# wg-perception/tod

Measured on AMD Instinct MI355X. Metric: frames/sec @ 640x480, 1M-descriptor DB; achieved HBM GB/s on BF-matcher, higher is better.
Workload: dtype fp4 (+-1) x fp4 -> f32 on the matrix cores (exact integers), f32 in the verifier

## Files before the change

tod_amd/csrc/orb.hip:

```cpp
#include <algorithm>
#include <cstring>
#include <vector>

#include "ctx.h"
#include "orb_arc.h"
#include "orb_compass.h"
#include "orb_stages.h"

using namespace tod_orb;

namespace {

#include "orb_pyramid.h"
#include "orb_fast.h"
#include "orb_select.h"
#include "orb_describe.h"

struct OrbGraph {
  struct Key { uint32_t H, W, n_features, n_levels, cap, F; float sf; const void *kp, *aux, *desc, *img0, *mask, *taps; } key = {};
  hipGraph_t graph = nullptr;
  hipGraphExec_t exec = nullptr;
  void drop() {
    if (exec) (void)hipGraphExecDestroy(exec);
    if (graph) (void)hipGraphDestroy(graph);
// ... 37 lines not shown
  TOD_HIP(ws->o_desc.reserve((size_t)P.F * P.cap * 32));
  if (masked) TOD_HIP(ws->maskbuf.reserve(P.F * P.px));
  TOD_HIP(ws->taps.reserve((size_t)P.n_taps * sizeof(ResizeTap) + 32));
  return TODHIP_OK;
}

int upload_pattern(todhip_ctx* ctx, OrbWs* ws, const int8_t* pattern) {
  if (!pattern && ws->pattern_is_default) return TODHIP_OK;
  int8_t hpat[1024];
  if (pattern) std::memcpy(hpat, pattern, 1024); else default_pattern(hpat);
  ws->pattern_is_default = !pattern;
  TOD_HIP(hipMemcpyAsync(ws->pattern.p, hpat, 1024, hipMemcpyHostToDevice, ctx->stream));
  TOD_HIP(hipStreamSynchronize(ctx->stream));
  return TODHIP_OK;
}

int upload_taps(todhip_ctx* ctx, OrbWs* ws, const OrbPlan& P, float scale_factor) {
  const OrbWs::TapsFor now = {P.H, P.W, P.n_levels, scale_factor, ws->taps.p};
  if (std::memcmp(&now, &ws->taps_for, sizeof(now)) == 0 || P.n_taps == 0u) return TODHIP_OK;
  std::vector<ResizeTap> taps(P.n_taps);
  fill_resize_taps(P, taps.data());
  TOD_HIP(hipMemcpyAsync(ws->taps.p, taps.data(), taps.size() * sizeof(ResizeTap), hipMemcpyHostToDevice, ctx->stream));
  TOD_HIP(hipStreamSynchronize(ctx->stream));
  ws->taps_for = now;
  return TODHIP_OK;
}

void record_stages(const OrbPlan& P, const OrbWs* ws, const uint8_t* d_mask, hipStream_t st) {
  const LevelTab& T = P.tab;
  const size_t px = P.px;
  for (uint32_t lvl = 1; lvl < P.n_levels; ++lvl) {
    if (P.resize_x[lvl] == 0u) continue;
    uint8_t* img = ws->pyr.as<uint8_t>() + (size_t)lvl * P.F * px;
    const ResizeTap* taps = ws->taps.as<ResizeTap>();
    hipLaunchKernelGGL(resize_kernel, grid(P.resize[lvl]), dim3(256), 0, st, img - (size_t)P.F * px, T.w[lvl - 1], img, T.h[lvl], T.w[lvl],
                       taps + P.tap_x[lvl], taps + P.tap_y[lvl], px);
  }
  uint32_t* ctl = ws->small.as<uint32_t>();
  uint32_t* level_counts = ctl + P.level_counts_off;
  Cand* cand = ws->cand.as<Cand>(); Cand* eq = ws->eq.as<Cand>(); Cand* sel1 = ws->sel1.as<Cand>(); Cand* sel2 = ws->sel2.as<Cand>();
  hipLaunchKernelGGL(fast_nms_kernel, grid(P.fast_nms), dim3(256), 0, st, T, cand, P.cand_cap, ctl, ctl + W_HIST, d_mask, P.H, P.W, px);
  hipLaunchKernelGGL(fast_threshold_kernel, grid(P.fast_threshold), dim3(64), 0, st, T, ctl, P.cand_cap);
  hipLaunchKernelGGL(split_kernel, grid(P.split), dim3(256), 0, st, T, cand, ctl, sel1, eq, P.cand_cap, P.sel1_cap);
  hipLaunchKernelGGL(rank_tiled_kernel, grid(P.rank_ties), dim3(256), 0, st, RankArgs::rank_ties(eq, P.cand_cap, sel1, P.sel1_cap, ctl));
  hipLaunchKernelGGL(harris_kernel, grid(P.harris), dim3(256), 0, st, T, sel1, ctl + W_NSEL1, px, P.sel1_cap);
  hipLaunchKernelGGL(rank_tiled_kernel, grid(P.rank_harris), dim3(256), 0, st,
                     RankArgs::rank_harris(sel1, P.sel1_cap, sel2, P.sel2_cap, ctl, level_counts, P.F));
  hipLaunchKernelGGL(blur_kernel, grid(P.blur), dim3(256), 0, st, T, ws->blur.as<uint8_t>(), px);
  DescribeArgs D;
  std::memset(&D, 0, sizeof(D));
  disc_umax(D.umax);
  D.blur = ws->blur.as<uint8_t>(); D.sel = sel2; D.level_counts = level_counts; D.cap = P.cap; D.pattern = ws->pattern.as<int8_t>();
  D.kp_xy = ws->o_xy.as<float>(); D.kp_aux = ws->o_aux.as<float>(); D.desc = ws->o_desc.as<uint8_t>(); D.fs = px; D.sel_fs = P.sel2_cap;
  hipLaunchKernelGGL(describe_kernel, grid(P.describe), dim3(256), 0, st, T, D);
}

int orb_device(todhip_ctx* ctx, const OrbIn& in, const OrbParams& par, const OrbOut& out) {
  OrbPlan P;
  if (const int bad = orb_plan(in.F, in.H, in.W, par.n_features, par.n_levels, par.scale_factor, out.cap, &P)) return bad;
  OrbWs* ws = tod_ws<OrbWs>(ctx);
  hipStream_t st = ctx->stream;
  if (P.want_max == 0) {
    ws->graph.drop();
    ws->plan = P;
    for (uint32_t f = 0; f < in.F; ++f) out.n_out[f] = 0;
    TOD_HIP(hipStreamSynchronize(st));
    return TODHIP_OK;
  }
  if (const int rc = reserve_buffers(ctx, ws, P, in.d_mask != nullptr)) return rc;
  if (const int rc = upload_pattern(ctx, ws, par.pattern)) return rc;
  if (const int rc = upload_taps(ctx, ws, P, par.scale_factor)) return rc;
  for (uint32_t lvl = 0; lvl < P.n_levels; ++lvl) P.tab.img[lvl] = ws->pyr.as<uint8_t>() + (size_t)lvl * P.F * P.px;
  ws->plan = P;
  uint32_t* ctl = ws->small.as<uint32_t>();
  TOD_HIP(hipMemsetAsync(ctl, 0, P.ctl_words * sizeof(uint32_t), st));
  if (in.stride == P.W && (P.F == 1 || in.gray_fs == P.px))
    TOD_HIP(hipMemcpyAsync(ws->pyr.p, in.d_gray, (size_t)P.F * P.px, hipMemcpyDeviceToDevice, st));
  else
    hipLaunchKernelGGL(copy_rows_kernel, grid(P.copy_rows), dim3(256), 0, st, in.d_gray, in.stride, ws->pyr.as<uint8_t>(), P.H, P.W,
                       in.gray_fs, P.px);
  const uint8_t* ws_mask = nullptr;
  if (in.d_mask) {
    ws_mask = ws->maskbuf.as<uint8_t>();
    hipLaunchKernelGGL(copy_rows_kernel, grid(P.copy_rows), dim3(256), 0, st, in.d_mask, P.W, ws->maskbuf.as<uint8_t>(), P.H, P.W, P.px, P.px);
  }
  float* const ws_xy = ws->o_xy.as<float>(); float* const ws_aux = ws->o_aux.as<float>(); uint8_t* const ws_desc = ws->o_desc.as<uint8_t>();
  static const bool use_graph = getenv("TODHIP_ORB_NO_GRAPH") == nullptr;
  if (!use_graph) {
    record_stages(ws->plan, ws, ws_mask, st);
  } else {
    const OrbGraph::Key key = {P.H, P.W, par.n_features, P.n_levels, P.cap, P.F, par.scale_factor, ws_xy, ws_aux, ws_desc, ws->pyr.p, ws_mask, ws->taps.p};
    if (!ws->graph.matches(key)) {
      TOD_HIP(ws->graph.begin_capture(st));
      record_stages(ws->plan, ws, ws_mask, st);
      TOD_HIP(ws->graph.end_capture(st, key));
    }
    TOD_HIP(ws->graph.launch(st));
  }
  uint32_t* d_totals = ctl + P.totals_off;
  hipLaunchKernelGGL(copy_out_kernel, grid(P.copy_out), dim3(256), 0, st, ctl + P.level_counts_off, P.n_levels, P.cap, ws_xy, ws_aux,
                     reinterpret_cast<const uint32_t*>(ws_desc), out.kp_xy, out.kp_aux, reinterpret_cast<uint32_t*>(out.desc), d_totals);
  TOD_HIP(hipGetLastError());
  uint32_t* h_totals = ws->h_out.as<uint32_t>();
  TOD_HIP(hipMemcpyAsync(h_totals, d_totals, (size_t)P.F * sizeof(uint32_t), hipMemcpyDeviceToHost, st));
  TOD_HIP(hipStreamSynchronize(st));
  for (uint32_t f = 0; f < P.F; ++f) out.n_out[f] = std::min(h_totals[f], P.cap);
  return TODHIP_OK;
// ... 113 lines not shown
```

tod_amd/csrc/orb_describe.h:

```cpp

struct DescribeArgs {
  const uint8_t* blur;
  const Cand* sel;
  const uint32_t* level_counts;
  uint32_t cap;
  const int8_t* pattern; int umax[kHalfPatch + 2];
  float* kp_xy; float* kp_aux; uint8_t* desc;
  size_t fs; uint32_t sel_fs;
};

__global__ __launch_bounds__(256) void describe_kernel(LevelTab T, const DescribeArgs A) {
  const uint32_t v = blockIdx.y, lvl = v / T.F, f = v - lvl * T.F;
  if (T.want[lvl] == 0u) return;
  const uint8_t* __restrict__ img = T.img[lvl] + f * A.fs;
  const uint8_t* __restrict__ blur = A.blur + v * A.fs;
  const Cand* __restrict__ sel = A.sel + (size_t)v * A.sel_fs;
  const uint32_t* __restrict__ level_counts = A.level_counts + f * kCtlWords;
  float* kp_xy = A.kp_xy + (size_t)f * A.cap * 2; float* kp_aux = A.kp_aux + (size_t)f * A.cap * 4;
  uint8_t* desc = A.desc + (size_t)f * A.cap * 32;
  const float scale = T.scale[lvl];
  const uint32_t i = blockIdx.x * 4u + (threadIdx.x >> 6), l = threadIdx.x & 63u;
  if (i >= level_counts[lvl]) return;
  uint32_t base = 0;
  for (uint32_t j = 0; j < lvl; ++j) base += level_counts[j];
  const uint32_t o = base + i;
  if (o >= A.cap) return;
  const Cand c = sel[i];
  const int x = c.x, y = c.y, W = (int)T.w[lvl];
  int m10, m01;
  patch_moments(img, W, x, y, A.umax, l, m10, m01);
  const float fm10 = (float)m10, fm01 = (float)m01;
  float ca, sa;
  steer_of(fm10, fm01, ca, sa);
  uint32_t nib = 0;
#pragma unroll
  for (int b = 0; b < 4; ++b) nib |= (uint32_t)steered_test(blur, W, x, y, ca, sa, A.pattern + 4 * (4 * (int)l + b)) << b;
  const uint32_t hi = __shfl_down(nib, 1);
  if ((l & 1u) == 0u) desc[(size_t)o * 32 + (l >> 1)] = (uint8_t)(nib | (hi << 4));
  if (l == 0) {
    float ang = atan2f(fm01, fm10) * 57.29577951308232f;
    if (ang < 0.f) ang += 360.f;
    kp_xy[2 * o] = (float)x * scale; kp_xy[2 * o + 1] = (float)y * scale;
    kp_aux[4 * o] = 31.f * scale; kp_aux[4 * o + 1] = ang; kp_aux[4 * o + 2] = c.harris; kp_aux[4 * o + 3] = (float)lvl;
  }
}

__global__ __launch_bounds__(256) void copy_out_kernel(const uint32_t* __restrict__ level_counts, uint32_t n_levels, uint32_t cap,
                                                       const float* __restrict__ s_xy, const float* __restrict__ s_aux,
                                                       const uint32_t* __restrict__ s_desc, float* __restrict__ d_xy,
                                                       float* __restrict__ d_aux, uint32_t* __restrict__ d_desc,
                                                       uint32_t* __restrict__ totals) {
  const uint32_t f = blockIdx.y;
  level_counts += f * kCtlWords;
  s_xy += (size_t)f * cap * 2; s_aux += (size_t)f * cap * 4; s_desc += (size_t)f * cap * 8;
  d_xy += (size_t)f * cap * 2; d_aux += (size_t)f * cap * 4; d_desc += (size_t)f * cap * 8;
  uint32_t total = 0;
  for (uint32_t l = 0; l < n_levels; ++l) total += level_counts[l];
  const uint32_t n = min(total, cap);
  const uint32_t i = blockIdx.x * 256u + threadIdx.x;
  if (i == 0) totals[f] = total;
  if (i < 2u * n) d_xy[i] = s_xy[i];
  if (i < 4u * n) d_aux[i] = s_aux[i];
  if (i < 8u * n) d_desc[i] = s_desc[i];
}
```

tod_amd/csrc/orb_stages.h:

```cpp
#pragma once

#include "ctx.h"
#include "orb_moments.h"
#include "orb_plan.h"

namespace tod_orb {

__device__ __forceinline__ uint32_t wave_append(uint32_t* counter, bool flag) {
  const uint32_t lane = threadIdx.x & 63u;
  const unsigned long long bal = __builtin_amdgcn_ballot_w64(flag);
  if (bal == 0ull) return 0u;
  const uint32_t first = (uint32_t)__ffsll((long long)bal) - 1u;
  uint32_t base = 0;
  if (lane == first) base = atomicAdd(counter, (uint32_t)__popcll(bal));
  base = (uint32_t)__builtin_amdgcn_readlane((int)base, (int)first);
  return base + (uint32_t)__popcll(bal & ((1ull << lane) - 1ull));
}

__device__ __forceinline__ uint32_t wave_prefix_sum(uint32_t v) {
#define TOD_ORB_DPP_ADD(ctrl, rows) v += (uint32_t)__builtin_amdgcn_update_dpp(0, (int)v, ctrl, rows, 0xF, false)
  TOD_ORB_DPP_ADD(0x111, 0xF); TOD_ORB_DPP_ADD(0x112, 0xF); TOD_ORB_DPP_ADD(0x114, 0xF); TOD_ORB_DPP_ADD(0x118, 0xF);
  TOD_ORB_DPP_ADD(0x142, 0xA); TOD_ORB_DPP_ADD(0x143, 0xC);
#undef TOD_ORB_DPP_ADD
  return v;
}
__device__ __forceinline__ uint32_t wave_sum(uint32_t v) { return (uint32_t)__builtin_amdgcn_readlane((int)wave_prefix_sum(v), 63); }

__device__ __forceinline__ void patch_moments(const uint8_t* __restrict__ img, int W, int x, int y, const int (&umax)[kHalfPatch + 2],
                                              uint32_t l, int& m10, int& m01) {
  m10 = 0; m01 = 0;
  if (l < 31u) {
    const int v = (int)l - kHalfPatch;
    const int d = v == 0 ? kHalfPatch : umax[v < 0 ? -v : v];
    int rs;
    row_moments(img + (size_t)(y + v) * W + x - kHalfPatch, d, rs, m10);
    m01 = v * rs;
  }
  m10 = (int)wave_sum((uint32_t)m10); m01 = (int)wave_sum((uint32_t)m01);
}

__device__ __forceinline__ void steer_of(float fm10, float fm01, float& ca, float& sa) {
  const float nrm = sqrtf(fm10 * fm10 + fm01 * fm01);
  ca = nrm > 0.f ? fm10 / nrm : 1.f; sa = nrm > 0.f ? fm01 / nrm : 0.f;
}

__device__ __forceinline__ bool steered_test(const uint8_t* __restrict__ blur, int W, int x, int y, float ca, float sa, const int8_t* pp) {
  const int x0 = (int)rintf((float)pp[0] * ca - (float)pp[1] * sa), y0 = (int)rintf((float)pp[0] * sa + (float)pp[1] * ca);
  const int x1 = (int)rintf((float)pp[2] * ca - (float)pp[3] * sa), y1 = (int)rintf((float)pp[2] * sa + (float)pp[3] * ca);
  const int t0 = blur[(uint32_t)(y + y0) * (uint32_t)W + (uint32_t)(x + x0)], t1 = blur[(uint32_t)(y + y1) * (uint32_t)W + (uint32_t)(x + x1)];
  return t0 < t1;
}

struct Stages {
  LevelTab T;
  const uint8_t* blur; const Cand* sel; const uint32_t* level_counts;
  size_t fs; uint32_t sel_fs, want_max, n;
  int umax[kHalfPatch + 2];
};

}

int tod_orb_stage_host_view(todhip_ctx* ctx, const uint8_t* gray, const uint8_t* mask, uint32_t H, uint32_t W, uint32_t stride,
                            const uint8_t** d_gray, const uint8_t** d_mask);
int tod_orb_stages(todhip_ctx* ctx, const uint8_t* d_gray, const uint8_t* d_mask, uint32_t H, uint32_t W, uint32_t stride,
                   uint32_t n_features, uint32_t n_levels, float scale_factor, tod_orb::Stages* out);
```

tod_amd/csrc/verify.hip:

```cpp
#include <algorithm>
#include <chrono>
#include <atomic>
#include <climits>
#include <cmath>
#include <cstdio>
#include <cstdlib>
#include <cstring>
#include <limits>
#include <map>
#include <memory>
#include <mutex>
#include <thread>
#include <vector>

#include "ctx.h"
#include "depth_rescale.h"
#include "verify_kernels.h"
#include "verify_draw_bits.h"

using namespace tod;

namespace {

#include "verify_launch.h"
#include "verify_prep.h"
#include "verify_draw.h"
#include "verify_clique.h"
#include "verify_eval.h"
#include "verify_growth.h"
#include "verify_sprint.h"


struct VerifyWs {
  DevBuf train, query, qidx, kpxy, phys, samp, bits, sampdeg, nvalid, table, iter_samples, counts, gate_m,
      small, deferred, stacks, kp_bits, clique_adj, adjc_scratch, c_kept, c_offs, c_qpt, c_obj, c_hist, c_goff,
      sprint_status, sprint_stack, c_src, c_cnt;
  HostBuf m_small, m_hist, m_pos, m_counts, m_kp, m_nvalid;
  HostBuf m_sprint, m_sprint_out, m_sprint_kp;
  HostBuf h_small;
};

struct StreamCache;
struct VerifyPool : TodWs {
  static constexpr int kSlot = kWsVerify;
  std::vector<VerifyWs*> slots; std::vector<StreamCache*> streams;
  std::vector<hipEvent_t> side_ev;
  static constexpr size_t kMaxLanes = 17;
  HostBuf args_stage[kMaxLanes]; DevBuf args_dev[kMaxLanes];
  DevBuf kceil; bool kceil_ready = false;
  ~VerifyPool() override;
};
struct SideStreams {
  struct PerDevice {
    std::vector<hipStream_t> st;
    std::atomic<bool> taken[16];
    uint32_t partition = 0;
    PerDevice() { for (auto& t : taken) t.store(false); }
  };
  std::mutex mu;
  std::map<int, PerDevice> by_device;
  hipError_t get(int device, uint32_t n, std::vector<hipStream_t>& out, PerDevice** pd) {
    std::lock_guard<std::mutex> g(mu);
    PerDevice& d = by_device[device];
    const uint32_t part = tod_cu_partition();
    if (d.partition != part) {
      bool in_use = false;
      for (size_t i = 0; i < d.st.size(); ++i) in_use = in_use || d.taken[i].load();
      if (!in_use) {
        for (hipStream_t s0 : d.st) { (void)hipStreamSynchronize(s0); (void)hipStreamDestroy(s0); }
        d.st.clear();
        d.partition = part;
// ... 410 lines not shown
```

tod_amd/csrc/verify_engine.h:

```cpp

enum Phase { PH_CLUSTER, PH_CLUSTER_WAIT, PH_PREPALL, PH_PREPALL_WAIT, PH_OBJECT, PH_ROUND, PH_PREP_WAIT, PH_DRAW,
             PH_DRAW_WAIT, PH_EVAL2, PH_EVAL2_WAIT, PH_GROWTH, PH_GROWTH_WAIT, PH_SPRINT_WAIT, PH_DONE };

struct RoundState {
  uint64_t consumed = 0;
  uint32_t it_drawn = 0, attempts_carry = 0;
  bool selection_empty = false, loop_done = false;
  int iterations = 0, n_best = -INT_MAX;
  double k = 1.0;
  uint32_t best_it = 0;
  uint64_t pos_after_stop = 0;
  uint32_t batch = 16, lookahead = 4096;
  uint32_t nvalid = 0, total_iters = 0;
  uint32_t it_begin = 0, want = 0, got = 0, S = 0, window_len = 0;
  uint32_t n_def = 0;
  uint32_t s_floor = 0;
};

inline uint64_t sprint_margin0() {
  static const uint64_t v = [] { const char* e = getenv("TODHIP_SPRINT_MARGIN"); const long long x = e ? atoll(e) : 0; return x > 0 ? (uint64_t)x : (uint64_t)(1u << 17); }();
  return v;
}
struct Slot {
  VerifyWs* ws = nullptr;
// ... 574 lines not shown
        for (uint32_t i = 0; i < n; ++i) { const dim3 e = extent(host[start[c] + i0 + i]); gx = std::max(gx, e.x); gy = std::max(gy, e.y); }
        const dim3 grid = slot_dim == 1 ? dim3(gx, n) : dim3(gx, gy, n);
        SlotsPtr<A> S = {dev + start[c] + i0};
        hipLaunchKernelGGL(kern, grid, dim3(block), lds, st, S);
      }
    }
    return true;
  }

  struct Staging { bool ok = false; size_t used = 0; };
  template <uint32_t N, class A, class KernP, class KernV, class Extent>
  void launch_either(hipStream_t st, KernP kern_ptr, KernV kern_val, const std::vector<A>& v, bool long_list, Staging& stage, int slot_dim,
                     Extent extent, uint32_t block, uint32_t lds, bool by_class) {
    if (long_list && stage.ok && launch_many(st, kern_ptr, v, slot_dim, extent, stage.used, block, lds, by_class)) return;
    launch_list<N>(st, kern_val, v, block, lds, slot_dim, extent);
  }
#define TOD_BOTH_FORMS(kern, A, N) kern<SlotsPtr<A>>, kern<Slots<A, N>>

  template <class F>
  static void split_evals(const std::vector<EvalArgs>& v, uint32_t lds, bool deferred, F& launch_evals) {
    bool any_wide = false, any_narrow = false;
    for (const EvalArgs& a : v) (a.job.W <= 8u ? any_narrow : any_wide) = true;
    if (any_wide && any_narrow) { launch_evals(v, true, lds, deferred); return; }
    launch_evals(v, any_wide, lds, deferred);
  }
  void launch_all(hipStream_t st) {
    Staging stage;
    {
      const size_t n_eval = L.eval_small.size() + L.eval_direct.size() + L.eval_big.size();
      if (L.adj.size() > 4u * kManySlots || n_eval > kMaxSlots || L.prep_small.size() > kManySlots) {
        VerifyPool* pool = tod_ws<VerifyPool>(ctx);
        const size_t need = L.finite.size() * sizeof(JobArgs) + L.adj.size() * sizeof(AdjArgs) + L.prep.size() * sizeof(PrepArgs) +
                            L.prep_small.size() * sizeof(PrepSmallArgs) + n_eval * sizeof(EvalArgs) + 4096u;
        stage.ok = pool->args_stage[lane_now].reserve(need) == hipSuccess && pool->args_dev[lane_now].reserve(need) == hipSuccess;
      }
    }
    auto launch_evals = [&](const std::vector<EvalArgs>& v, bool wide, uint32_t lds, bool deferred) {
      pick_eval(wide, deferred, [&](auto kern_ptr, auto kern_val, auto ext) {
        launch_either<kMaxSlots>(st, kern_ptr, kern_val, v, v.size() > kMaxSlots, stage, 1, ext, 64u, lds, false);
      });
    };
    auto words = [](const CopyArgs& a) { return dim3(std::max(1u, std::min(64u, (a.n + 255u) / 256u))); };
    L.copy_in.insert(L.copy_in.end(), L.zero.begin(), L.zero.end());
    launch_list<kCopySlots>(st, copy_words_kernel, L.copy_in, 256, 0, 1, words);
    for (size_t i = 0; i < L.sprint.size(); ++i) { L.sprint[i].rnd = L.sprint_src[i]->dev.as<uint32_t>(); L.sprint[i].rnd_len = L.sprint_src[i]->dev_valid; }
    launch_list<kWideSlots>(st, sprint_kernel, L.sprint, kSprintThreads, kSprintLds, 0, [](const SprintArgs&) { return dim3(1); });
    launch_list(st, cluster_frame_kernel, L.cluster, 256, 0, 0, [](const ClusterArgs&) { return dim3(1); });
    launch_list(st, cluster_frame_rescaled_kernel, L.cluster_rescaled, 256, 0, 0, [](const ClusterRescaledArgs&) { return dim3(1); });
    launch_list<kWideSlots>(st, invalidate_kernel, L.inval, 256, 0, 0, [](const InvArgs&) { return dim3(1); });
    launch_either<kManySlots>(st, TOD_BOTH_FORMS(small_prep_kernel, PrepSmallArgs, kManySlots), L.prep_small, L.prep_small.size() > kManySlots, stage,
                              1, [](const PrepSmallArgs&) { return dim3(1); }, 64u, 0u, false);
    {
      auto ext_rows = [](const auto& a) { return dim3((a.job.n + 255u) / 256u); };
      auto ext_adj = [](const AdjArgs& a) { return dim3(a.job.n, (a.job.W + 3u) / 4u); };
      const bool many = L.adj.size() > 4u * kManySlots;
      launch_either<kManySlots>(st, TOD_BOTH_FORMS(finite_kernel, JobArgs, kManySlots), L.finite, many, stage, 1, ext_rows, 256u, 0u, true);
      launch_either<kManySlots>(st, TOD_BOTH_FORMS(adjacency_kernel, AdjArgs, kManySlots), L.adj, many, stage, 2, ext_adj, 256u, 0u, true);
      launch_either<kManySlots>(st, TOD_BOTH_FORMS(round_prep_kernel, PrepArgs, kManySlots), L.prep, many, stage, 1, ext_rows, 256u, 0u, true);
    }
    for (int f = DRAW_FORMS - 1; f >= 0; --f) {
      for (size_t i = 0; i < L.draw[f].size(); ++i) L.draw[f][i].rnd = L.draw_src[f][i].first->dev.as<uint32_t>() + L.draw_src[f][i].second;
      launch_draws(st, (DrawForm)f, L.draw[f]);
    }
    {
      uint32_t lds = 0;
      for (const ChainArgs& c : L.chain) lds = std::max(lds, (std::min(c.S, kChainLdsEntries) + std::min(c.n_req, kChainMaxReq)) * 4u);
      launch_list<kWideSlots>(st, chain_kernel, L.chain, 256, lds, 0, [](const ChainArgs&) { return dim3(1); });
    }
    {
      uint32_t lds = 8192u;
      for (const EvalArgs& a : L.eval_small) lds = std::max(lds, a.lds_bytes);
      for (EvalArgs& a : L.eval_small) a.lds_bytes = lds;
      split_evals(L.eval_small, lds, false, launch_evals);
    }
    split_evals(L.eval_direct, kEvalLdsBig, false, launch_evals);
    split_evals(L.eval_big, kEvalLdsBig, true, launch_evals);
    launch_list(st, growth_kernel, L.growth, 256, 0, 0, [](const GrowthArgs&) { return dim3(1); });
    launch_list<kWideSlots>(st, invalidate_kernel, L.inval_after, 256, 0, 0, [](const InvArgs&) { return dim3(1); });
    launch_list<kManySlots>(st, round_prep_kernel<Slots<PrepArgs, kManySlots>>, L.prep_after, 256, 0, 1, [](const PrepArgs& a) { return dim3((a.job.n + 255u) / 256u); });
    launch_list<kCopySlots>(st, copy_words_kernel, L.copy_out, 256, 0, 1, words);
    L = Launches();
  }
#undef TOD_BOTH_FORMS

  int run(std::vector<Slot*>& slots) {
    std::vector<StreamCache*>& caches = tod_ws<VerifyPool>(ctx)->streams;
    for (Slot* s : slots) {
      s->start_draws = s->rng->draws; s->abs_pos = 0; s->stream = nullptr;
      for (StreamCache* c : caches) if (c->same_start(*s->rng)) { s->stream = c; break; }
      if (!s->stream) {
        if (caches.size() >= 64) {
          bool in_use = false;
          for (Slot* t : slots) in_use = in_use || t->stream == caches.front();
          if (!in_use) { TOD_HIP(hipStreamSynchronize(st)); caches.front()->dev.release(); delete caches.front(); caches.erase(caches.begin()); }
        }
        caches.push_back(new StreamCache(*s->rng));
        s->stream = caches.back();
      }
    }
    const int rc_run = run_ticks(slots);
    for (Slot* s : slots) {
      if (s->abs_pos) { const uint64_t d0 = s->start_draws; *s->rng = s->stream->state_at(s->abs_pos); s->rng->draws = d0 + s->abs_pos; }
      s->stream = nullptr;
    }
    return rc_run;
  }
  static constexpr uint32_t kHeavyN = 96;
  enum Kind { K_LIGHT = 0, K_GROWTH = 1, K_SPRINT = 2, K_EVAL = 3, K_COUNT = 4 };
  static Kind kind_of(const Slot& s) {
    if (s.ph == PH_OBJECT) {
// ... 119 lines not shown
```

tod_amd/csrc/verify_hooks.h:

```cpp

namespace {
struct LookupArgs { const float* kp_xy; const void* depth; float* z; uint32_t* err; uint32_t n, H, W; int is_u16, rescale; RescaleGeom geom; };
__global__ __launch_bounds__(256) void depth_lookup_kernel(LookupArgs a) {
  const uint32_t q = blockIdx.x * 256u + threadIdx.x;
  if (q >= a.n) return;
  const int row = (int)a.kp_xy[2 * q + 1], col = (int)a.kp_xy[2 * q];
  if (row < 0 || col < 0 || (uint32_t)row >= a.H || (uint32_t)col >= a.W) { atomicExch(a.err, 1u); return; }
  a.z[q] = a.rescale ? rescaled_depth_at(a.depth, a.is_u16, a.geom, (uint32_t)col, (uint32_t)row)
                     : depth_metres(a.depth, a.is_u16, (size_t)row * a.W + col);
}
__global__ __launch_bounds__(64) void kabsch_test_kernel(uint32_t n, const double* Hd, const float* C, float* R, float* T) {
  const uint32_t i = blockIdx.x * 64u + threadIdx.x;
  if (i >= n) return;
  double h[9]; float c[6], r[9], t[3];
  for (int k = 0; k < 9; ++k) h[k] = Hd[(size_t)i * 9 + k];
  for (int k = 0; k < 6; ++k) c[k] = C[(size_t)i * 6 + k];
  kabsch_solve(h, c, r, t);
  for (int k = 0; k < 9; ++k) R[(size_t)i * 9 + k] = r[k];
  for (int k = 0; k < 3; ++k) T[(size_t)i * 3 + k] = t[k];
}
}

extern "C" {

int todhip_test_kabsch(todhip_ctx* ctx, uint32_t n_cases, const double* Hd, const float* C, float* R, float* T) {
  if (!ctx || !Hd || !C || !R || !T || n_cases == 0 || n_cases > (1u << 20)) return TODHIP_EINVAL;
  TOD_HIP(hipSetDevice(ctx->device));
  VerifyWs* ws = ws_of(ctx);
  hipStream_t st = ctx->stream;
  const size_t n = n_cases;
  TOD_HIP(ws->phys.reserve(n * 9 * sizeof(double))); TOD_HIP(ws->train.reserve(n * 6 * sizeof(float)));
  TOD_HIP(ws->query.reserve(n * 9 * sizeof(float))); TOD_HIP(ws->kpxy.reserve(n * 3 * sizeof(float)));
  TOD_HIP(hipMemcpyAsync(ws->phys.p, Hd, n * 9 * sizeof(double), hipMemcpyHostToDevice, st));
  TOD_HIP(hipMemcpyAsync(ws->train.p, C, n * 6 * sizeof(float), hipMemcpyHostToDevice, st));
  hipLaunchKernelGGL(kabsch_test_kernel, dim3((n_cases + 63u) / 64u), dim3(64), 0, st, n_cases, ws->phys.as<double>(),
                     ws->train.as<float>(), ws->query.as<float>(), ws->kpxy.as<float>());
  TOD_HIP(hipGetLastError());
  TOD_HIP(hipMemcpyAsync(R, ws->query.p, n * 9 * sizeof(float), hipMemcpyDeviceToHost, st));
  TOD_HIP(hipMemcpyAsync(T, ws->kpxy.p, n * 3 * sizeof(float), hipMemcpyDeviceToHost, st));
  TOD_HIP(hipStreamSynchronize(st));
  return TODHIP_OK;
}

int todhip_test_adjacency(todhip_ctx* ctx, const float* train, const float* query, const float* kpxy, uint32_t n,
                          float span, float err, uint64_t* phys, uint64_t* samp) {
  if (!ctx || !train || !query || !kpxy || !phys || !samp || n == 0 || n > (uint32_t)kMaxWords * 64u) return TODHIP_EINVAL;
  TOD_HIP(hipSetDevice(ctx->device));
  VerifyWs* ws = ws_of(ctx);
  const uint32_t W = (n + 63u) / 64u;
  hipStream_t st = ctx->stream;
  TOD_HIP(ws->train.reserve((size_t)n * 12)); TOD_HIP(ws->query.reserve((size_t)n * 12));
  TOD_HIP(ws->kpxy.reserve((size_t)n * 8));
  TOD_HIP(ws->phys.reserve((size_t)n * W * 8)); TOD_HIP(ws->samp.reserve((size_t)n * W * 8));
  TOD_HIP(ws->bits.reserve((size_t)8 * W * 8));
  TOD_HIP(hipMemcpyAsync(ws->train.p, train, (size_t)n * 12, hipMemcpyHostToDevice, st));
  TOD_HIP(hipMemcpyAsync(ws->query.p, query, (size_t)n * 12, hipMemcpyHostToDevice, st));
  TOD_HIP(hipMemcpyAsync(ws->kpxy.p, kpxy, (size_t)n * 8, hipMemcpyHostToDevice, st));
  ObjJob job;
  std::memset(&job, 0, sizeof(job));
  job.n = n; job.W = W;
  job.train = ws->train.as<float>(); job.query = ws->query.as<float>(); job.kpxy = ws->kpxy.as<float>();
  job.phys = ws->phys.as<u64>(); job.samp = ws->samp.as<u64>();
  launch_list<kManySlots>(st, adjacency_kernel<Slots<AdjArgs, kManySlots>>, std::vector<AdjArgs>{{job, span, err}}, 256, 0, 2,
              [](const AdjArgs& a) { return dim3(a.job.n, (a.job.W + 3u) / 4u); });
  TOD_HIP(hipGetLastError());
  TOD_HIP(hipMemcpyAsync(phys, ws->phys.p, (size_t)n * W * 8, hipMemcpyDeviceToHost, st));
  TOD_HIP(hipMemcpyAsync(samp, ws->samp.p, (size_t)n * W * 8, hipMemcpyDeviceToHost, st));
  TOD_HIP(hipStreamSynchronize(st));
  return TODHIP_OK;
}

int todhip_test_consensus(todhip_ctx* ctx, const float* train, const float* query, const float* kpxy, uint32_t n,
                          float span, float err, const uint32_t* triples, uint32_t n_triples, uint32_t stop_level,
                          int32_t* counts, uint32_t* dbg, uint32_t dbg_stride) {
  if (!ctx || !train || !query || !kpxy || !triples || !counts || n < 3 || n > (uint32_t)kMaxWords * 64u || n_triples == 0)
    return TODHIP_EINVAL;
  TOD_HIP(hipSetDevice(ctx->device));
  int rc = set_big_lds_once(ctx);
  if (rc != TODHIP_OK) return rc;
  VerifyWs* ws = ws_of(ctx);
  const uint32_t W = (n + 63u) / 64u;
  hipStream_t st = ctx->stream;
  TOD_HIP(ws->train.reserve((size_t)n * 12)); TOD_HIP(ws->query.reserve((size_t)n * 12));
  TOD_HIP(ws->qidx.reserve((size_t)n * 4)); TOD_HIP(ws->kpxy.reserve((size_t)n * 8));
  TOD_HIP(ws->phys.reserve((size_t)n * W * 8)); TOD_HIP(ws->samp.reserve((size_t)n * W * 8));
  TOD_HIP(ws->bits.reserve((size_t)8 * W * 8)); TOD_HIP(ws->sampdeg.reserve((size_t)n * 4));
  TOD_HIP(ws->small.reserve(256 * sizeof(uint32_t))); TOD_HIP(ws->h_small.reserve(256 * sizeof(uint32_t)));
  TOD_HIP(ws->iter_samples.reserve((size_t)n_triples * 12)); TOD_HIP(ws->counts.reserve((size_t)n_triples * 4));
  TOD_HIP(ws->gate_m.reserve((size_t)n_triples * 4)); TOD_HIP(ws->deferred.reserve((size_t)n_triples * 4));
  TOD_HIP(ws->stacks.reserve((size_t)kMaxEvalWaves * kStackCap * sizeof(uint16_t)));
  if (dbg) TOD_HIP(ws->table.reserve((size_t)n_triples * dbg_stride * 4));
  TOD_HIP(hipMemcpyAsync(ws->train.p, train, (size_t)n * 12, hipMemcpyHostToDevice, st));
  TOD_HIP(hipMemcpyAsync(ws->query.p, query, (size_t)n * 12, hipMemcpyHostToDevice, st));
  TOD_HIP(hipMemcpyAsync(ws->kpxy.p, kpxy, (size_t)n * 8, hipMemcpyHostToDevice, st));
  TOD_HIP(hipMemcpyAsync(ws->iter_samples.p, triples, (size_t)n_triples * 12, hipMemcpyHostToDevice, st));
  TOD_HIP(hipMemsetAsync(ws->qidx.p, 0, (size_t)n * 4, st));
  if (dbg) TOD_HIP(hipMemsetAsync(ws->table.p, 0, (size_t)n_triples * dbg_stride * 4, st));
  ObjJob job;
  job.n = n; job.W = W;
  job.train = ws->train.as<float>(); job.query = ws->query.as<float>(); job.qidx = ws->qidx.as<uint32_t>();
  job.kpxy = ws->kpxy.as<float>(); job.phys = ws->phys.as<u64>(); job.samp = ws->samp.as<u64>();
  u64* bits = ws->bits.as<u64>();
  job.finite = bits; job.valid = bits + W; job.deg7 = bits + 2 * W; job.sampdeg = ws->sampdeg.as<uint32_t>();
  SlotCtl* d_ctl = ws->small.as<SlotCtl>();
  EvalStatus* h_eval = &ws->h_small.as<SlotCtl>()->eval;
  TOD_HIP(hipMemsetAsync(d_ctl, 0, sizeof(SlotCtl), st));
  launch_list<kManySlots>(st, finite_kernel<Slots<JobArgs, kManySlots>>, std::vector<JobArgs>{{job}}, 256, 0, 1, [](const JobArgs& a) { return dim3((a.job.n + 255u) / 256u); });
  launch_list<kManySlots>(st, adjacency_kernel<Slots<AdjArgs, kManySlots>>, std::vector<AdjArgs>{{job, span, err}}, 256, 0, 2,
              [](const AdjArgs& a) { return dim3(a.job.n, (a.job.W + 3u) / 4u); });
  launch_list<kManySlots>(st, round_prep_kernel<Slots<PrepArgs, kManySlots>>, std::vector<PrepArgs>{{job, d_ctl->prep, nullptr, 0u}}, 256, 0, 1,
              [](const PrepArgs& a) { return dim3((a.job.n + 255u) / 256u); });
  EvalArgs A = eval_args(job, ws, ws->counts.as<int32_t>(), 0u, n_triples, kEvalLdsSmall);
  A.dbg = dbg ? ws->table.as<uint32_t>() : nullptr; A.dbg_stride = dbg_stride; A.stop_level = stop_level;
  if (n_triples > kMaxEvalWaves) return TODHIP_EINVAL;
  auto launch = [&](auto, auto kern, auto ext) { launch_list(st, kern, std::vector<EvalArgs>{A}, 64, A.lds_bytes, 1, ext); };
  pick_eval(W > 8u, false, launch);
  TOD_HIP(hipGetLastError());
  TOD_HIP(hipMemcpyAsync(h_eval, &d_ctl->eval, sizeof(EvalStatus), hipMemcpyDeviceToHost, st));
  TOD_HIP(hipStreamSynchronize(st));
  const uint32_t status = h_eval->error, n_def = h_eval->n_deferred;
  if (status == 0 && n_def > 0) {
    A.lds_bytes = kEvalLdsBig; A.from_deferred = 1; A.n_deferred = n_def;
    TOD_HIP(ws->adjc_scratch.reserve((size_t)n_def * kAdjcScratchWords * sizeof(u64)));
    A.adjc_scratch = ws->adjc_scratch.as<u64>();
    TOD_HIP(hipMemsetAsync(&d_ctl->eval_work, 0, sizeof(uint32_t), st));
    pick_eval(W > 8u, true, launch);
    TOD_HIP(hipGetLastError());
    TOD_HIP(hipMemcpyAsync(h_eval, &d_ctl->eval, sizeof(EvalStatus), hipMemcpyDeviceToHost, st));
    TOD_HIP(hipStreamSynchronize(st));
  }
  TOD_HIP(hipMemcpyAsync(counts, ws->counts.p, (size_t)n_triples * 4, hipMemcpyDeviceToHost, st));
  if (dbg) TOD_HIP(hipMemcpyAsync(dbg, ws->table.p, (size_t)n_triples * dbg_stride * 4, hipMemcpyDeviceToHost, st));
  TOD_HIP(hipStreamSynchronize(st));
  if (h_eval->error != 0) {
    TOD_DBG("consensus status %u: g=%u value=%u m=%u it=%u", h_eval->error, h_eval->detail_g, h_eval->detail_value, h_eval->detail_m, h_eval->detail_it);
    return TODHIP_ESCRATCH;
  }
  return TODHIP_OK;
}

int todhip_test_draw_table(todhip_ctx* ctx, const uint64_t* samp, const uint64_t* valid, uint32_t n, const uint32_t* rnd,
                           uint32_t window_len, uint32_t S, uint32_t form, uint32_t* entries_out) {
  if (!ctx || !samp || !valid || !rnd || !entries_out || n == 0 || n > (uint32_t)kMaxWords * 64u || S == 0 || S > (1u << 20) ||
      window_len == 0 || window_len > (1u << 24) || form > 4u)
    return TODHIP_EINVAL;
  const uint32_t W = (n + 63u) / 64u;
  DrawForm f = draw_form_of(W);
  if (form == 1u) f = W <= 2u ? DRAW_LANE2 : DRAW_LANE8;
  if (form == 2u) f = DRAW_WAVE1;
  if (form == 3u) f = DRAW_WAVE8;
  if (form == 4u) f = DRAW_LANE8;
  if (W > draw_form_max_words(f)) return TODHIP_EINVAL;
  TOD_HIP(hipSetDevice(ctx->device));
  VerifyWs* ws = ws_of(ctx);
  hipStream_t st = ctx->stream;
  TOD_HIP(ws->samp.reserve((size_t)n * W * 8)); TOD_HIP(ws->bits.reserve((size_t)8 * W * 8));
  TOD_HIP(ws->iter_samples.reserve((size_t)window_len * 4));
  TOD_HIP(ws->table.reserve((size_t)S * sizeof(DrawEntry)));
  TOD_HIP(hipMemcpyAsync(ws->samp.p, samp, (size_t)n * W * 8, hipMemcpyHostToDevice, st));
  TOD_HIP(hipMemcpyAsync(ws->bits.as<u64>() + W, valid, (size_t)W * 8, hipMemcpyHostToDevice, st));
  TOD_HIP(hipMemcpyAsync(ws->iter_samples.p, rnd, (size_t)window_len * 4, hipMemcpyHostToDevice, st));
  TOD_HIP(hipMemsetAsync(ws->table.p, 0xFF, (size_t)S * sizeof(DrawEntry), st));
// ... 79 lines not shown
```

tod_amd/csrc/verify_prep.h:

```cpp

struct AdjArgs { ObjJob job; float span, err; };
struct JobArgs { ObjJob job; };
struct PrepArgs { ObjJob job; uint32_t* stats; const uint32_t* gate; uint32_t gate_min; };

__device__ __forceinline__ void pair_test(const float* q1, const float* q2, const float* t1, const float* t2, const float* k1, const float* k2,
                                          float span, float err, bool& phys, bool& samp) {
  phys = false; samp = false;
  float dq = dist_sq3(q1, q2);
  const float lim = (span + 2 * err) * (span + 2 * err);
  if (!(dq > lim)) {
    dq = sqrtf(dq);
    const float dt = (float)norm3d(t1[0] - t2[0], t1[1] - t2[1], t1[2] - t2[2]);
    const float a = fabsf(dt - dq);
    if (!(a > 4 * err)) {
      phys = true;
      const float px = (k1[0] - k2[0]) * (k1[0] - k2[0]) + (k1[1] - k2[1]) * (k1[1] - k2[1]);
      samp = (px > 20 * 20) && (a < 2 * err);
    }
  }
}

template <class H>
__global__ __launch_bounds__(256) void adjacency_kernel(H S) {
  TOD_LATENCY_PRIO();
  const ObjJob& job = S.a[blockIdx.z].job;
  const float span = S.a[blockIdx.z].span, err = S.a[blockIdx.z].err;
  const uint32_t i = blockIdx.x;
  if (i >= job.n) return;
  const uint32_t word = blockIdx.y * 4u + (threadIdx.x >> 6);
  if (word >= job.W) return;
  const uint32_t j = word * 64u + lane_id();
  bool phys = false, samp = false;
  if (j < job.n && j != i) {
    const uint32_t lo = min(i, j), hi = max(i, j);
    pair_test(job.query + 3 * lo, job.query + 3 * hi, job.train + 3 * lo, job.train + 3 * hi, job.kpxy + 2 * lo, job.kpxy + 2 * hi, span, err,
              phys, samp);
  }
  const u64 pb = __ballot(phys), sb = __ballot(samp);
  if (lane_id() == 0) {
    job.phys[(size_t)i * job.W + word] = pb;
    job.samp[(size_t)i * job.W + word] = sb;
  }
}

template <class H>
__global__ __launch_bounds__(256) void finite_kernel(H S) {
  TOD_LATENCY_PRIO();
  const ObjJob& job = S.a[blockIdx.y].job;
  const uint32_t v = blockIdx.x * 256u + threadIdx.x;
  bool f = false;
  if (v < job.n) {
    f = true;
    for (int c = 0; c < 3; ++c) f = f && isfinite(job.train[3 * v + c]) && isfinite(job.query[3 * v + c]);
  }
  const u64 b = __ballot(f);
  const uint32_t word = v >> 6;
  if (lane_id() == 0 && word < job.W) {
    job.finite[word] = b;
    const uint32_t base = word * 64u;
    job.valid[word] = base + 64u <= job.n ? ~0ull : (base < job.n ? ((1ull << (job.n - base)) - 1ull) : 0ull);
  }
}

template <class H>
__global__ __launch_bounds__(256) void round_prep_kernel(H S) {
  TOD_LATENCY_PRIO();
  const ObjJob& job = S.a[blockIdx.y].job;
  uint32_t* const stats = S.a[blockIdx.y].stats;
  if (S.a[blockIdx.y].gate && *S.a[blockIdx.y].gate < S.a[blockIdx.y].gate_min) return;
  const uint32_t v = blockIdx.x * 256u + threadIdx.x;
  bool isv = false;
  uint32_t d = 0;
  if (v < job.n) {
    isv = (job.valid[v >> 6] >> (v & 63u)) & 1ull;
    if (isv)
      for (uint32_t w = 0; w < job.W; ++w) d += (uint32_t)__popcll(job.samp[(size_t)v * job.W + w] & job.valid[w]);
    job.sampdeg[v] = d;
  }
  const u64 b7 = __ballot(isv && d >= kGateMinimal), bv = __ballot(isv);
  const uint32_t dsum = wave_sum(d);
  if (lane_id() == 0 && (v >> 6) < job.W) {
    job.deg7[v >> 6] = b7;
    if (bv) atomicAdd(stats, (uint32_t)__popcll(bv));
    if (dsum) atomicAdd(stats + 1, dsum);
  }
  if (isv && d >= 2u) {
    const u64* rv = job.samp + (size_t)v * job.W;
    for (uint32_t wj = v >> 6; wj < job.W; ++wj) {
      u64 nb = rv[wj] & job.valid[wj];
      if (wj == (v >> 6)) nb &= (v & 63u) == 63u ? 0ull : ~0ull << ((v & 63u) + 1u);
      while (nb) {
        if (__hip_atomic_load(stats + 2, __ATOMIC_RELAXED, __HIP_MEMORY_SCOPE_AGENT) != 0u) return;
        const uint32_t j = wj * 64u + (uint32_t)__ffsll((long long)nb) - 1u;
        nb &= nb - 1ull;
        const u64* rj = job.samp + (size_t)j * job.W;
// ... 220 lines not shown
```

Before: 25680.

## Halve describe waves per keypoint and tile symmetric adjacency computation

```diff
diff --git a/tod_amd/csrc/orb.hip b/tod_amd/csrc/orb.hip
--- a/tod_amd/csrc/orb.hip
+++ b/tod_amd/csrc/orb.hip
@@ -113,7 +113,7 @@
   disc_umax(D.umax);
   D.blur = ws->blur.as<uint8_t>(); D.sel = sel2; D.level_counts = level_counts; D.cap = P.cap; D.pattern = ws->pattern.as<int8_t>();
   D.kp_xy = ws->o_xy.as<float>(); D.kp_aux = ws->o_aux.as<float>(); D.desc = ws->o_desc.as<uint8_t>(); D.fs = px; D.sel_fs = P.sel2_cap;
-  hipLaunchKernelGGL(describe_kernel, grid(P.describe), dim3(256), 0, st, T, D);
+  hipLaunchKernelGGL(describe_kernel, grid(P.describe), dim3(kDescribeThreads), 0, st, T, D);
 }
 
 int orb_device(todhip_ctx* ctx, const OrbIn& in, const OrbParams& par, const OrbOut& out) {
diff --git a/tod_amd/csrc/orb_describe.h b/tod_amd/csrc/orb_describe.h
--- a/tod_amd/csrc/orb_describe.h
+++ b/tod_amd/csrc/orb_describe.h
@@ -9,7 +9,8 @@
   size_t fs; uint32_t sel_fs;
 };
 
-__global__ __launch_bounds__(256) void describe_kernel(LevelTab T, const DescribeArgs A) {
+constexpr uint32_t kDescribeThreads = 128;
+__global__ __launch_bounds__(kDescribeThreads) void describe_kernel(LevelTab T, const DescribeArgs A) {
   const uint32_t v = blockIdx.y, lvl = v / T.F, f = v - lvl * T.F;
   if (T.want[lvl] == 0u) return;
   const uint8_t* __restrict__ img = T.img[lvl] + f * A.fs;
@@ -19,25 +20,30 @@
   float* kp_xy = A.kp_xy + (size_t)f * A.cap * 2; float* kp_aux = A.kp_aux + (size_t)f * A.cap * 4;
   uint8_t* desc = A.desc + (size_t)f * A.cap * 32;
   const float scale = T.scale[lvl];
-  const uint32_t i = blockIdx.x * 4u + (threadIdx.x >> 6), l = threadIdx.x & 63u;
-  if (i >= level_counts[lvl]) return;
+  const uint32_t l = threadIdx.x & 63u, hl = l & 31u, count = level_counts[lvl];
+  const uint32_t i0 = (uint32_t)__builtin_amdgcn_readfirstlane((int)(blockIdx.x * 4u + (threadIdx.x >> 6) * 2u));
+  if (i0 >= count) return;
   uint32_t base = 0;
   for (uint32_t j = 0; j < lvl; ++j) base += level_counts[j];
-  const uint32_t o = base + i;
-  if (o >= A.cap) return;
+  if (base + i0 >= A.cap) return;
+  const uint32_t both = (i0 + 1u < count && base + i0 + 1u < A.cap) ? 1u : 0u;
+  const uint32_t i = i0 + ((l >> 5) & both), o = base + i;
+  const bool live = both != 0u || l < 32u;
   const Cand c = sel[i];
   const int x = c.x, y = c.y, W = (int)T.w[lvl];
   int m10, m01;
-  patch_moments(img, W, x, y, A.umax, l, m10, m01);
+  patch_moments_half(img, W, x, y, A.umax, hl, m10, m01);
   const float fm10 = (float)m10, fm01 = (float)m01;
   float ca, sa;
   steer_of(fm10, fm01, ca, sa);
-  uint32_t nib = 0;
+  uint32_t bits = 0;
+#pragma unroll 1
+  for (int n = 0; n < 8; n += 4) {
 #pragma unroll
-  for (int b = 0; b < 4; ++b) nib |= (uint32_t)steered_test(blur, W, x, y, ca, sa, A.pattern + 4 * (4 * (int)l + b)) << b;
-  const uint32_t hi = __shfl_down(nib, 1);
-  if ((l & 1u) == 0u) desc[(size_t)o * 32 + (l >> 1)] = (uint8_t)(nib | (hi << 4));
-  if (l == 0) {
+    for (int b = 0; b < 4; ++b) bits |= (uint32_t)steered_test(blur, W, x, y, ca, sa, A.pattern + 4 * (8 * (int)hl + n + b)) << (n + b);
+  }
+  if (live) desc[(size_t)o * 32 + hl] = (uint8_t)bits;
+  if (live && hl == 0) {
     float ang = atan2f(fm01, fm10) * 57.29577951308232f;
     if (ang < 0.f) ang += 360.f;
     kp_xy[2 * o] = (float)x * scale; kp_xy[2 * o + 1] = (float)y * scale;
diff --git a/tod_amd/csrc/orb_stages.h b/tod_amd/csrc/orb_stages.h
--- a/tod_amd/csrc/orb_stages.h
+++ b/tod_amd/csrc/orb_stages.h
@@ -17,17 +17,22 @@
   return base + (uint32_t)__popcll(bal & ((1ull << lane) - 1ull));
 }
 
+#define TOD_ORB_DPP_ADD(ctrl, rows) v += (uint32_t)__builtin_amdgcn_update_dpp(0, (int)v, ctrl, rows, 0xF, false)
 __device__ __forceinline__ uint32_t wave_prefix_sum(uint32_t v) {
-#define TOD_ORB_DPP_ADD(ctrl, rows) v += (uint32_t)__builtin_amdgcn_update_dpp(0, (int)v, ctrl, rows, 0xF, false)
   TOD_ORB_DPP_ADD(0x111, 0xF); TOD_ORB_DPP_ADD(0x112, 0xF); TOD_ORB_DPP_ADD(0x114, 0xF); TOD_ORB_DPP_ADD(0x118, 0xF);
   TOD_ORB_DPP_ADD(0x142, 0xA); TOD_ORB_DPP_ADD(0x143, 0xC);
-#undef TOD_ORB_DPP_ADD
   return v;
 }
 __device__ __forceinline__ uint32_t wave_sum(uint32_t v) { return (uint32_t)__builtin_amdgcn_readlane((int)wave_prefix_sum(v), 63); }
+__device__ __forceinline__ uint32_t half_wave_sum(uint32_t v) {
+  TOD_ORB_DPP_ADD(0x111, 0xF); TOD_ORB_DPP_ADD(0x112, 0xF); TOD_ORB_DPP_ADD(0x114, 0xF); TOD_ORB_DPP_ADD(0x118, 0xF);
+  TOD_ORB_DPP_ADD(0x142, 0xA);
+  return (uint32_t)__builtin_amdgcn_ds_bpermute((int)(((threadIdx.x & 63u) | 31u) << 2), (int)v);
+}
+#undef TOD_ORB_DPP_ADD
 
-__device__ __forceinline__ void patch_moments(const uint8_t* __restrict__ img, int W, int x, int y, const int (&umax)[kHalfPatch + 2],
-                                              uint32_t l, int& m10, int& m01) {
+__device__ __forceinline__ void patch_row(const uint8_t* __restrict__ img, int W, int x, int y, const int (&umax)[kHalfPatch + 2],
+                                          uint32_t l, int& m10, int& m01) {
   m10 = 0; m01 = 0;
   if (l < 31u) {
     const int v = (int)l - kHalfPatch;
@@ -36,7 +41,16 @@
     row_moments(img + (size_t)(y + v) * W + x - kHalfPatch, d, rs, m10);
     m01 = v * rs;
   }
+}
+__device__ __forceinline__ void patch_moments(const uint8_t* __restrict__ img, int W, int x, int y, const int (&umax)[kHalfPatch + 2],
+                                              uint32_t l, int& m10, int& m01) {
+  patch_row(img, W, x, y, umax, l, m10, m01);
   m10 = (int)wave_sum((uint32_t)m10); m01 = (int)wave_sum((uint32_t)m01);
+}
+__device__ __forceinline__ void patch_moments_half(const uint8_t* __restrict__ img, int W, int x, int y, const int (&umax)[kHalfPatch + 2],
+                                                   uint32_t hl, int& m10, int& m01) {
+  patch_row(img, W, x, y, umax, hl, m10, m01);
+  m10 = (int)half_wave_sum((uint32_t)m10); m01 = (int)half_wave_sum((uint32_t)m01);
 }
 
 __device__ __forceinline__ void steer_of(float fm10, float fm01, float& ca, float& sa) {
diff --git a/tod_amd/csrc/verify.hip b/tod_amd/csrc/verify.hip
--- a/tod_amd/csrc/verify.hip
+++ b/tod_amd/csrc/verify.hip
@@ -17,6 +17,7 @@
 #include "depth_rescale.h"
 #include "verify_kernels.h"
 #include "verify_draw_bits.h"
+#include "verify_adj_tiles.h"
 
 using namespace tod;
 
diff --git a/tod_amd/csrc/verify_adj_tiles.h b/tod_amd/csrc/verify_adj_tiles.h
--- /dev/null
+++ b/tod_amd/csrc/verify_adj_tiles.h
@@ -0,0 +1,26 @@
+#pragma once
+#include <cstdint>
+
+#if defined(__HIPCC__)
+#define TOD_ADJ_HD __host__ __device__ __forceinline__
+#else
+#define TOD_ADJ_HD inline
+#endif
+
+namespace tod {
+
+constexpr uint32_t kAdjTileWaves = 4;
+constexpr uint32_t kAdjWaveRows = 64 / kAdjTileWaves;
+
+TOD_ADJ_HD uint32_t adj_tile_count(uint32_t W) { return W * (W + 1u) / 2u; }
+
+TOD_ADJ_HD void adj_tile_decode(uint32_t t, uint32_t& I, uint32_t& J) {
+  uint32_t j = (uint32_t)((__builtin_sqrtf((float)(8u * t + 1u)) - 1.f) * 0.5f);
+  while (j * (j + 1u) / 2u > t) --j;
+  while ((j + 1u) * (j + 2u) / 2u <= t) ++j;
+  I = t - j * (j + 1u) / 2u; J = j;
+}
+
+TOD_ADJ_HD uint64_t adj_col_halfword(uint32_t j, uint32_t W, uint32_t I, uint32_t w) { return ((uint64_t)j * W + I) * 4u + w; }
+
+}
diff --git a/tod_amd/csrc/verify_engine.h b/tod_amd/csrc/verify_engine.h
--- a/tod_amd/csrc/verify_engine.h
+++ b/tod_amd/csrc/verify_engine.h
@@ -650,10 +650,11 @@
                               1, [](const PrepSmallArgs&) { return dim3(1); }, 64u, 0u, false);
     {
       auto ext_rows = [](const auto& a) { return dim3((a.job.n + 255u) / 256u); };
-      auto ext_adj = [](const AdjArgs& a) { return dim3(a.job.n, (a.job.W + 3u) / 4u); };
       const bool many = L.adj.size() > 4u * kManySlots;
       launch_either<kManySlots>(st, TOD_BOTH_FORMS(finite_kernel, JobArgs, kManySlots), L.finite, many, stage, 1, ext_rows, 256u, 0u, true);
-      launch_either<kManySlots>(st, TOD_BOTH_FORMS(adjacency_kernel, AdjArgs, kManySlots), L.adj, many, stage, 2, ext_adj, 256u, 0u, true);
+      launch_adjacency([&](auto kern_ptr, auto kern_val, int slot_dim, auto extent, uint32_t block, uint32_t lds) {
+        launch_either<kManySlots>(st, kern_ptr, kern_val, L.adj, many, stage, slot_dim, extent, block, lds, true);
+      });
       launch_either<kManySlots>(st, TOD_BOTH_FORMS(round_prep_kernel, PrepArgs, kManySlots), L.prep, many, stage, 1, ext_rows, 256u, 0u, true);
     }
     for (int f = DRAW_FORMS - 1; f >= 0; --f) {
diff --git a/tod_amd/csrc/verify_hooks.h b/tod_amd/csrc/verify_hooks.h
--- a/tod_amd/csrc/verify_hooks.h
+++ b/tod_amd/csrc/verify_hooks.h
@@ -61,8 +61,9 @@
   job.n = n; job.W = W;
   job.train = ws->train.as<float>(); job.query = ws->query.as<float>(); job.kpxy = ws->kpxy.as<float>();
   job.phys = ws->phys.as<u64>(); job.samp = ws->samp.as<u64>();
-  launch_list<kManySlots>(st, adjacency_kernel<Slots<AdjArgs, kManySlots>>, std::vector<AdjArgs>{{job, span, err}}, 256, 0, 2,
-              [](const AdjArgs& a) { return dim3(a.job.n, (a.job.W + 3u) / 4u); });
+  launch_adjacency([&](auto, auto kern_val, int slot_dim, auto extent, uint32_t block, uint32_t lds) {
+    launch_list<kManySlots>(st, kern_val, std::vector<AdjArgs>{{job, span, err}}, block, lds, slot_dim, extent);
+  });
   TOD_HIP(hipGetLastError());
   TOD_HIP(hipMemcpyAsync(phys, ws->phys.p, (size_t)n * W * 8, hipMemcpyDeviceToHost, st));
   TOD_HIP(hipMemcpyAsync(samp, ws->samp.p, (size_t)n * W * 8, hipMemcpyDeviceToHost, st));
@@ -106,8 +107,9 @@
   EvalStatus* h_eval = &ws->h_small.as<SlotCtl>()->eval;
   TOD_HIP(hipMemsetAsync(d_ctl, 0, sizeof(SlotCtl), st));
   launch_list<kManySlots>(st, finite_kernel<Slots<JobArgs, kManySlots>>, std::vector<JobArgs>{{job}}, 256, 0, 1, [](const JobArgs& a) { return dim3((a.job.n + 255u) / 256u); });
-  launch_list<kManySlots>(st, adjacency_kernel<Slots<AdjArgs, kManySlots>>, std::vector<AdjArgs>{{job, span, err}}, 256, 0, 2,
-              [](const AdjArgs& a) { return dim3(a.job.n, (a.job.W + 3u) / 4u); });
+  launch_adjacency([&](auto, auto kern_val, int slot_dim, auto extent, uint32_t block, uint32_t lds) {
+    launch_list<kManySlots>(st, kern_val, std::vector<AdjArgs>{{job, span, err}}, block, lds, slot_dim, extent);
+  });
   launch_list<kManySlots>(st, round_prep_kernel<Slots<PrepArgs, kManySlots>>, std::vector<PrepArgs>{{job, d_ctl->prep, nullptr, 0u}}, 256, 0, 1,
               [](const PrepArgs& a) { return dim3((a.job.n + 255u) / 256u); });
   EvalArgs A = eval_args(job, ws, ws->counts.as<int32_t>(), 0u, n_triples, kEvalLdsSmall);
diff --git a/tod_amd/csrc/verify_prep.h b/tod_amd/csrc/verify_prep.h
--- a/tod_amd/csrc/verify_prep.h
+++ b/tod_amd/csrc/verify_prep.h
@@ -20,27 +20,74 @@
   }
 }
 
+__device__ __forceinline__ float rdlane_f(float v, uint32_t lane) { return __uint_as_float(rdlane(__float_as_uint(v), lane)); }
+template <bool kDiag>
+__device__ __forceinline__ void adjacency_tile_rows(const float* __restrict__ query, const float* __restrict__ train, const float* __restrict__ kpxy,
+                                                    u64* __restrict__ phys, u64* __restrict__ samp, uint32_t n, uint32_t W, uint32_t I, uint32_t J,
+                                                    uint32_t w, float span, float err) {
+  const uint32_t l = lane_id(), j = J * 64u + l;
+  float qj[3] = {0.f, 0.f, 0.f}, tj[3] = {0.f, 0.f, 0.f}, kj[2] = {0.f, 0.f};
+  if (j < n) {
+    for (int c = 0; c < 3; ++c) { qj[c] = query[3 * j + c]; tj[c] = train[3 * j + c]; }
+    kj[0] = kpxy[2 * j]; kj[1] = kpxy[2 * j + 1];
+  }
+  const uint32_t i0 = I * 64u + w * kAdjWaveRows;
+  float qr[3] = {0.f, 0.f, 0.f}, tr[3] = {0.f, 0.f, 0.f}, kr[2] = {0.f, 0.f};
+  if (l < kAdjWaveRows && i0 + l < n) {
+    const uint32_t i = i0 + l;
+    for (int c = 0; c < 3; ++c) { qr[c] = query[3 * i + c]; tr[c] = train[3 * i + c]; }
+    kr[0] = kpxy[2 * i]; kr[1] = kpxy[2 * i + 1];
+  }
+  uint32_t pcol = 0u, scol = 0u;
+#pragma unroll 1
+  for (uint32_t r = 0; r < kAdjWaveRows; ++r) {
+    const uint32_t i = i0 + r;
+    if (kDiag && i >= n) break;
+    float qi[3], ti[3], ki[2];
+    for (int c = 0; c < 3; ++c) { qi[c] = rdlane_f(qr[c], r); ti[c] = rdlane_f(tr[c], r); }
+    ki[0] = rdlane_f(kr[0], r); ki[1] = rdlane_f(kr[1], r);
+    bool ph = false, sa = false;
+    if (j < n && (!kDiag || j != i)) {
+      if (kDiag) {
+        const bool sw = j < i;
+        float qa[3], qb[3], ta[3], tb[3], ka[2], kb[2];
+        for (int c = 0; c < 3; ++c) { qa[c] = sw ? qj[c] : qi[c]; qb[c] = sw ? qi[c] : qj[c]; ta[c] = sw ? tj[c] : ti[c]; tb[c] = sw ? ti[c] : tj[c]; }
+        for (int c = 0; c < 2; ++c) { ka[c] = sw ? kj[c] : ki[c]; kb[c] = sw ? ki[c] : kj[c]; }
+        pair_test(qa, qb, ta, tb, ka, kb, span, err, ph, sa);
+      } else {
+        pair_test(qi, qj, ti, tj, ki, kj, span, err, ph, sa);
+      }
+    }
+    const u64 pb = __ballot(ph), sb = __ballot(sa);
+    if (l == 0u) {
+      phys[(size_t)i * W + J] = pb;
+      samp[(size_t)i * W + J] = sb;
+    }
+    if (!kDiag) { pcol |= (uint32_t)ph << r; scol |= (uint32_t)sa << r; }
+  }
+  if (!kDiag && j < n) {
+    reinterpret_cast<uint16_t*>(phys)[adj_col_halfword(j, W, I, w)] = (uint16_t)pcol;
+    reinterpret_cast<uint16_t*>(samp)[adj_col_halfword(j, W, I, w)] = (uint16_t)scol;
+  }
+}
+
 template <class H>
-__global__ __launch_bounds__(256) void adjacency_kernel(H S) {
+__global__ __launch_bounds__(256) void adjacency_tile_kernel(H S) {
   TOD_LATENCY_PRIO();
   const ObjJob& job = S.a[blockIdx.z].job;
   const float span = S.a[blockIdx.z].span, err = S.a[blockIdx.z].err;
-  const uint32_t i = blockIdx.x;
-  if (i >= job.n) return;
-  const uint32_t word = blockIdx.y * 4u + (threadIdx.x >> 6);
-  if (word >= job.W) return;
-  const uint32_t j = word * 64u + lane_id();
-  bool phys = false, samp = false;
-  if (j < job.n && j != i) {
-    const uint32_t lo = min(i, j), hi = max(i, j);
-    pair_test(job.query + 3 * lo, job.query + 3 * hi, job.train + 3 * lo, job.train + 3 * hi, job.kpxy + 2 * lo, job.kpxy + 2 * hi, span, err,
-              phys, samp);
-  }
-  const u64 pb = __ballot(phys), sb = __ballot(samp);
-  if (lane_id() == 0) {
-    job.phys[(size_t)i * job.W + word] = pb;
-    job.samp[(size_t)i * job.W + word] = sb;
-  }
+  const uint32_t n = job.n, W = job.W;
+  if (blockIdx.x >= adj_tile_count(W)) return;
+  uint32_t I, J;
+  adj_tile_decode(blockIdx.x, I, J);
+  const uint32_t w = uni(threadIdx.x >> 6);
+  if (I == J) adjacency_tile_rows<true>(job.query, job.train, job.kpxy, job.phys, job.samp, n, W, I, J, w, span, err);
+  else adjacency_tile_rows<false>(job.query, job.train, job.kpxy, job.phys, job.samp, n, W, I, J, w, span, err);
+}
+template <class Launch>
+void launch_adjacency(Launch&& launch) {
+  launch(adjacency_tile_kernel<SlotsPtr<AdjArgs>>, adjacency_tile_kernel<Slots<AdjArgs, kManySlots>>, 2,
+         [](const AdjArgs& a) { return dim3(adj_tile_count(a.job.W)); }, 256u, 0u);
 }
 
 template <class H>
```

Result: no change. 25780, median of 6 (+0.4%).
